# TORlN/HDR-to-SDR

Hardware: AMD Instinct MI355X
Metric: Mpixel/s HDR10->SDR (4K frames) at 1/2/4/8 GPUs; % HBM roofline (higher is better)
Workload: dtype f32

## Files before the change

hdr-to-sdr_amd/csrc/h2s_tile.h:

```cpp
#pragma once
#include "h2s_tile_io.h"

namespace h2s {

__device__ __forceinline__ CurveConsts curve_of(const CurveConsts* frames, int f) {
  typedef __attribute__((address_space(4))) const float cfloat;
  constexpr int n = (int)(sizeof(CurveConsts) / sizeof(float));
  cfloat* src = (cfloat*)frames + __builtin_amdgcn_readfirstlane(f) * n;
  CurveConsts r;
  float* dst = reinterpret_cast<float*>(&r);
#pragma unroll
  for (int i = 0; i < n; i++) dst[i] = src[i];
  return r;
}

constexpr int TILE_WPE = 5;
constexpr int TILE_WPE_LP = TILE_WPE;

template <int TRC, int TM, int DESAT, int LP, int DBG = 0, bool SEMI = false, int SUB = 0>
__global__ __launch_bounds__(256) __attribute__((amdgpu_waves_per_eu(LP ? TILE_WPE_LP : TILE_WPE))) void k_tile(
    const FastParams F) {
  static_assert(DBG == 0 || DBG == 1, "the stage is F.dbg_stage, not a template value");
  static_assert(SUB == 0 || SUB == 3 || (LP == 0 && DBG == 0), "4:2:2 / 4:4:4 input: CPU chain product instances only");
  static_assert(SUB != 3 || (DBG == 0 && SEMI), "top-left 4:2:0 input: the SEMI product instances");
  constexpr bool S420 = SUB == 0 || SUB == 3;
  constexpr int YST = row_stride<LP>(), HST = YST;
  static_assert(TBH * C422_ST <= (CBH + 2) * HST && TBH * C444_ST <= 2 * (CBH + 2) * HST, "hrow holds the SUB windows");
  __shared__ __attribute__((aligned(16))) unsigned char yin[YIN_BYTES];
  __shared__ float hrow[2][(CBH + 2) * HST];
  __shared__ float csum[2][CBH * CBW];
  __shared__ float4 pq_lds[PQ_NSEG + 1];
  __shared__ float4 pqi_lds[LP ? PQI_NTAB : 1];
  extern __shared__ uint16_t eq_lds[];
  __shared__ int tflag[2];
  __shared__ int offtab[4];
  __shared__ unsigned spread_lds[LP ? 256 : 1];
  constexpr int ESC = TRC == 0 || !LP ? PQ_SEG : 1;

  const int t = threadIdx.x;
  const int lane = t & 63, w = t >> 6;
  const unsigned ntiles = F.nbx * F.nby * F.nframes;
  unsigned tile = (unsigned)xcd_remap(blockIdx.x, gridDim.x) * (unsigned)F.tpb;
  const unsigned tend = tile + (unsigned)F.tpb < ntiles ? tile + (unsigned)F.tpb : ntiles;

  TileGeo geo = tile_geo(F, tile);
  const LaneOfs lofs = lane_ofs<SEMI>(F, t);
  TileRegs<SEMI, SUB> cur = tile_load<SEMI, SUB>(F, geo, t, lofs);
  const __amdgpu_buffer_rsrc_t req = __builtin_amdgcn_make_buffer_rsrc((void*)F.eq_lut, (short)0, 2 * F.eq_n, 0x00020000);
  const unsigned eq0 = __builtin_amdgcn_raw_buffer_load_b16(req, 2 * t, 0, 0);
  float4 pq0 = make_float4(0.0f, 0.0f, 0.0f, 0.0f);
  const bool stage_pq = TRC != 1 || !LP || F.lp_ipt;
  if (stage_pq && t < PQ_NSEG) {
    const __amdgpu_buffer_rsrc_t rpq = __builtin_amdgcn_make_buffer_rsrc((void*)F.pq_tab, (short)0, 16 * PQ_NSEG, 0x00020000);
    pq0 = __builtin_bit_cast(float4, __builtin_amdgcn_raw_buffer_load_b128(rpq, 16 * t, 0, 0));
  }
  const int eq_sh = SEMI ? F.out_sh : 0;
  if (t < F.eq_n) eq_lds[t] = (uint16_t)(((eq0 << F.shift_out) | (eq0 >> F.rep_rs)) << eq_sh);
  for (int i = t + 256; i < F.eq_n; i += 256) {
    const unsigned v = __builtin_amdgcn_raw_buffer_load_b16(req, 2 * i, 0, 0);
    eq_lds[i] = (uint16_t)(((v << F.shift_out) | (v >> F.rep_rs)) << eq_sh);
  }
  if (stage_pq && t < PQ_NSEG)
    pq_lds[t + 1] = (TRC == 0 || LP) && t == 0 ? make_float4(0.0f, 0.0f, 3.40282347e38f, 0.0f) : pq0;
  if (stage_pq && t == 255) pq_lds[0] = make_float4(0.0f, 0.0f, 0.0f, 0.0f);
  if (t < 2) tflag[t] = 0;
  if (t < 3) offtab[t] = t == 0 ? 12 : (t == 1 ? F.og : F.ob);
  if (LP) {
    unsigned x = (unsigned)t;
    x = (x | (x << 8)) & 0x0F00Fu;
    x = (x | (x << 4)) & 0x0C30C3u;
    spread_lds[t] = (x | (x << 2)) & 0x249249u;
  }
  __syncthreads();
  if (LP && (F.lp_ipt || TRC == 2)) {
    const __amdgpu_buffer_rsrc_t rpi = __builtin_amdgcn_make_buffer_rsrc((void*)F.pqi_tab, (short)0, 16 * PQI_NTAB, 0x00020000);
    for (int i = t; i < PQI_NTAB; i += 256)
      pqi_lds[i] = __builtin_bit_cast(float4, __builtin_amdgcn_raw_buffer_load_b128(rpi, 16 * i, 0, 0));
  }

  const int qx = (lane >> 2) & 3, qy = lane >> 4, pxl = lane & 1, pyl = (lane >> 1) & 1;
  const int xl = 16 * w + 2 * qx + pxl, yl = 2 * qy + pyl;
  uint16_t* ybase = reinterpret_cast<uint16_t*>(yin + luma_at(xl, yl));
  const float* h0 = hrow[0] + (qy + 1) * HST + xl;
  const float* h1 = hrow[1] + (qy + 1) * HST + xl;
  const int hb = SUB == 3 ? (pyl ? HST : 0) : (pyl ? HST : -HST);
  const float* c0 = hrow[0] + yl * C422_ST + (xl >> 1);
  const float* c1 = hrow[1] + yl * C422_ST + (xl >> 1);
  const int16_t* s0 = reinterpret_cast<const int16_t*>(hrow[0]) + yl * C444_ST + xl;
  const int16_t* s1 = reinterpret_cast<const int16_t*>(hrow[1]) + yl * C444_ST + xl;
  float* csb = csum[0] + qy * CBW + 8 * w + qx;

  const float yoff = in_vgpr(F.y_off_c) * (float)ESC + (ESC == PQ_SEG ? 1.0f : 0.0f);
  const float cmid = in_vgpr(F.c_mid);
  const float a_rv = in_vgpr(F.a_rv[1]) * (float)ESC, a_gv = in_vgpr(F.a_gv[1]) * (float)ESC,
              a_gu = in_vgpr(F.a_gu[1]) * (float)ESC, a_bu = in_vgpr(F.a_bu[1]) * (float)ESC;
  const float stride_g = in_vgpr(F.stride_g), stride_b = in_vgpr(F.stride_b);
  const int og = in_vgpr(F.og), ob = in_vgpr(F.ob), ocr = in_vgpr(F.cr), ocg = in_vgpr(F.cg), ocb = in_vgpr(F.cb);
  const float log2_nm1 = in_vgpr(F.log2_nm1), x_max = in_vgpr(F.x_max);
  const float ysc = in_vgpr(F.ys) * (float)ESC;
  const float ydq = F.dither ? dither_off(xl, yl) - 0.5f : 0.0f;
  const StepK K{a_rv, a_gv, a_gu, a_bu, stride_g, stride_b, og, ob, ocr, ocg, ocb, log2_nm1, x_max,
                TM == 5 && !LP ? in_vgpr(F.hable_kb) : F.hable_kb, F.c111, rintf(1.0f / F.inv_nm1), offtab,
                LP ? in_vgpr(F.lp_k2) : 0.0f, LP ? in_vgpr(F.lp_k2 + 255.0f) : 0.0f, LP ? F.lp_cy + ydq : 0.0f,
                LP ? in_vgpr(F.lp_k1) : 0.0f};
  gu32* lut8v = LP ? in_vgpr64(F.lut8x) : nullptr;
  float qo[4];
#pragma unroll
  for (int i = 0; i < 4; i++)
    qo[i] = LP ? F.lp_qo + (F.lp_dith ? bayer16(xl + 8 * (i & 1), yl + 8 * (i >> 1)) : 0.5f) -
                     (F.lut_off ? 0.0f : F.lp_k2 * F.lp_qs_f)
               : 0.5f;

  auto steps = [&](const TileGeo& g, auto fast) {
    constexpr bool FB = decltype(fast)::value;
    constexpr int YR2 = YROW / 2;
    if constexpr (FB) {
      H2S_MARK("body: fast");
    } else {
      H2S_MARK("body: exact-capable");
    }
    CurveConsts cv = F;
    if ((TM == 7 || TM == 8 || LP) && F.cv_frames) cv = curve_of(F.cv_frames, g.f);
    const CDoviRec* const dv =
        TRC == 2 ? (const CDoviRec*)F.dovi + __builtin_amdgcn_readfirstlane(F.dovi_n == 1 ? 0 : F.dovi_f0 + g.f) : nullptr;
    if constexpr (LP && TM == 7) {
      cv.b_e1b = in_vgpr(cv.b_e1b), cv.b_tb = in_vgpr(cv.b_tb), cv.b_c2 = in_vgpr(cv.b_c2);
      cv.b_lc = in_vgpr(cv.b_lc), cv.b_bk_b = in_vgpr(cv.b_bk_b), cv.b_bk_d = in_vgpr(cv.b_bk_d);
    } else if constexpr (LP && TM == 8) {
      cv.sp_qb_u = in_vgpr(cv.sp_qb_u), cv.sp_pb_u = in_vgpr(cv.sp_pb_u);
      cv.sp_srcmax = in_vgpr(cv.sp_srcmax), cv.sp_umax = in_vgpr(cv.sp_umax);
    }
    const __amdgpu_buffer_rsrc_t lut = __builtin_amdgcn_make_buffer_rsrc((void*)F.lut_yuv, (short)0, F.lut_bytes, 0x00020000);
    const int live = !FB && DBG == 0 && !F.chr444 ? F.H - g.py0 : TBH;
    auto chroma_out = [&](int s, float oyv, float ozv) {
      if (!FB && F.chr444) {
        const int px = g.px0 + xl + 8 * (s & 1), py = g.py0 + yl + 8 * (s >> 1);
        F.chr444[(long long)py * F.chr_w + px] = make_float2(oyv * F.inv_c56, ozv * F.inv_c56);
        return;
      }
      H2S_MARK("S6 chroma quad sums");
      const int oc = 4 * (s >> 1) * CBW + 4 * (s & 1);
      const float su = quad_sum(oyv), sv = quad_sum(ozv);
      csb[oc] = su;
      csb[oc + CBH * CBW] = sv;
    };
    if constexpr (LP && DBG == 0) {
      if (!F.lut_off) {
        unsigned vp = 0;
#pragma unroll
        for (int s = 0; s <= 8; s++) {
          unsigned vn = 0;
          if (s < 8 && (FB || 8 * (s >> 1) < live)) {
            const int oy = 8 * (s >> 1) * YR2 + 8 * (s & 1);
            const int oh = 4 * (s >> 1) * HST + 8 * (s & 1);
            H2S_MARK("S0 step: staged Y, vertical chroma");
            const float ybs = fmaf((float)ybase[oy], ysc, yoff);
            const float U = SUB == 3 ? 2.0f * (h0[oh] + h0[oh + hb]) : fmaf(3.0f, h0[oh], h0[oh + hb]);
            const float V = SUB == 3 ? 2.0f * (h1[oh] + h1[oh + hb]) : fmaf(3.0f, h1[oh], h1[oh + hb]);
            float r, gg, bl;
            lin_tone<TRC, TM, DESAT, LP, 0, FB>(F, cv, pq_lds, pqi_lds, K, ybs, U, V, [](float, float, float) {},
                                                 r, gg, bl, dv);
            H2S_MARK("S3 encode");
            vn = lp_table_read(F, K, lut8v, spread_lds, r, gg, bl, qo[s & 3]);
          }
          if (s > 0 && (FB || 8 * ((s - 1) >> 1) < live)) {
            const int sp = s - 1;
            const float R8 = (float)(vp & 255u), G8 = (float)((vp >> 8) & 255u), B8 = (float)((vp >> 16) & 255u);
            H2S_MARK("S5 Y'CbCr");
            const f3 o = lp_ycbcr(F, K, R8, G8, B8);
            H2S_MARK("S7 eq");
            ybase[8 * (sp >> 1) * YR2 + 8 * (sp & 1)] = eq_lds[(int)o.x];
            chroma_out(sp, o.y, o.z);
          }
          vp = vn;
        }
        return;
      }
      H2S_MARK("body: lut off");
    }
#pragma unroll
    for (int s = 0; s < 8; s++) {
      if (!FB && (s & 1) == 0 && 8 * (s >> 1) >= live) break;
      const int oy = 8 * (s >> 1) * YR2 + 8 * (s & 1);
      const int oh = 4 * (s >> 1) * HST + 8 * (s & 1);
      H2S_MARK("S0 step: staged Y, vertical chroma");
      const float ybs = fmaf((float)ybase[oy], ysc, yoff);
      float U, V;
      if constexpr (SUB == 1) {
        const int oc = 8 * (s >> 1) * C422_ST + 4 * (s & 1);
        U = 4.0f * (c0[oc] + c0[oc + pxl]), V = 4.0f * (c1[oc] + c1[oc + pxl]);
      } else if constexpr (SUB == 2) {
        const int oc = 8 * (s >> 1) * C444_ST + 8 * (s & 1);
        U = 8.0f * (float)s0[oc], V = 8.0f * (float)s1[oc];
      } else if constexpr (SUB == 3) {
        U = 2.0f * (h0[oh] + h0[oh + hb]), V = 2.0f * (h1[oh] + h1[oh + hb]);
      } else {
        U = fmaf(3.0f, h0[oh], h0[oh + hb]);
        V = fmaf(3.0f, h1[oh], h1[oh + hb]);
      }
      const long long di = DBG && g.f == 0 && g.py0 + yl + 8 * (s >> 1) < F.H
                               ? (long long)(g.py0 + yl + 8 * (s >> 1)) * F.dbg_w + g.px0 + xl + 8 * (s & 1)
                               : -1;
      float oyv, ozv;
      ybase[oy] = (uint16_t)px_chain<TRC, TM, DESAT, LP, DBG, FB>(
          F, cv, pq_lds, pqi_lds, eq_lds, lut8v, spread_lds, lut, K, ybs, U, V, di, oyv, ozv, LP ? qo[s & 3] : 0.5f, ydq, dv);
      chroma_out(s, oyv, ozv);
    }
  };
  auto mask_in = [&](uint4& a) {
    a.x &= F.in_mask2, a.y &= F.in_mask2, a.z &= F.in_mask2, a.w &= F.in_mask2;
  };
  auto shift_in = [&](uint4& a) { a.x >>= F.in_sh, a.y >>= F.in_sh, a.z >>= F.in_sh, a.w >>= F.in_sh; };

  const int pl = __builtin_amdgcn_readfirstlane(t >> 6) & 1, rem = t & 63;
  const bool cst = t < 128 && !F.chr444;
  auto commit = [&](unsigned ti) {
    H2S_MARK("tile: commit");
    if constexpr (SEMI && S420) {
      if (!F.in_semi) cur.uh = halo_half(F, geo, t, cur.uh);
    }
    if (F.in_mask2 != 0xFFFFFFFFu) {
      if constexpr (SEMI && S420) {
        if (F.in_sh) {
          shift_in(cur.ya), shift_in(cur.ua);
          cur.uh >>= F.in_sh;
        }
      }
      mask_in(cur.ya), mask_in(cur.ua);
      if constexpr (SUB == 2) mask_in(cur.va);
      else cur.uh &= F.in_mask2;
    }
    const float my = stage_luma(yin, cur.ya, t >> 3, t & 7, ysc, yoff);
    float mc = 0.0f;
    if constexpr (SUB == 1) {
      mc = stage_chroma422(hrow[__builtin_amdgcn_readfirstlane(t >> 7)], cur.ua, cur.uh, t & 127, cmid);
    } else if constexpr (SUB == 2) {
      mc = stage_chroma444(hrow[0], hrow[1], cur.ua, cur.va, t >> 3, t & 7, (int)F.c_mid);
    } else if (SEMI && F.in_semi) {
      if (t < 144) mc = stage_chroma_semi<HST>(hrow[0], hrow[1], cur.ua, cur.uh, t, cmid);
    } else if ((t & 127) < 72) {
      mc = stage_chroma<HST>(hrow[__builtin_amdgcn_readfirstlane(t >> 7)], cur.ua, cur.uh, t & 127, cmid);
    }
    if constexpr (SUB == 2) asm volatile("" ::"v"(cur.ua.w), "v"(cur.va.w));
    else asm volatile("" ::"v"(cur.ua.w), "v"(cur.uh));
    if ((my > F.safe_y || mc > F.safe_c)) tflag[ti & 1u] = 1;
  };
  commit(tile);
  for (;;) {
    H2S_MARK("tile: prefetch");
    const int par = (int)(tile & 1u);
    const TileGeo g = geo;
    const bool more = tile + 1 < tend;
    if (more) {
      tile_next(F, geo);
      cur = tile_load<SEMI, SUB>(F, geo, t, lofs);
    }
    __syncthreads();
    const bool fb = __builtin_amdgcn_readfirstlane(tflag[par]) == 0 && !F.chr444 && !(DBG == 0 && g.py0 + TBH > F.H);
    if (t == 0) tflag[par ^ 1] = 0;
    if (fb)
      steps(g, std::integral_constant<bool, true>{});
    else
      steps(g, std::integral_constant<bool, false>{});
    H2S_MARK("tile: store");
    __syncthreads();

    put_luma(F, g, read_luma(F, yin, t >> 3, t & 7), t >> 3, lofs.sy, t);
    const bool osemi = SEMI && F.out_semi;
    u4v cv{0u, 0u, 0u, 0u};
    int cvo = ST_DROP;
    if (cst) {
      const int cr = osemi ? t >> 3 : rem >> 2;
      cv = osemi ? read_chroma_semi(F, csum[0], cr, t & 7) : read_chroma(F, csum[0], pl, cr, rem & 3);
      if (g.cy0 + cr < F.ch) cvo = lofs.sc;
    }
    put_chroma(F, g, cv, osemi ? 0 : pl, osemi, cvo, t);
    if (!more) break;
    commit(++tile);
  }
}

}
```

hdr-to-sdr_amd/csrc/h2s_tile_io.h:

```cpp
#pragma once
#include "h2s_tile_px.h"

namespace h2s {

constexpr int CBW = 32, CBH = 16;
constexpr int ROW_STRIDE = 72, ROW_STRIDE_LP = 68;
template <int LP>
constexpr int row_stride() { return LP ? ROW_STRIDE_LP : ROW_STRIDE; }
constexpr int AUX_NT = 2;
constexpr int NT = AUX_NT, NTS = AUX_NT;

__device__ __forceinline__ void unpack8(const uint4 a, float* o) {
  o[0] = (float)(a.x & 0xffff), o[1] = (float)(a.x >> 16), o[2] = (float)(a.y & 0xffff), o[3] = (float)(a.y >> 16);
  o[4] = (float)(a.z & 0xffff), o[5] = (float)(a.z >> 16), o[6] = (float)(a.w & 0xffff), o[7] = (float)(a.w >> 16);
}

__device__ __forceinline__ __amdgpu_buffer_rsrc_t plane_rsrc(const uint8_t* base, int bytes) {
  return __builtin_amdgcn_make_buffer_rsrc((void*)base, (short)0, bytes, 0x00020000);
}

template <bool SEMI, int SUB = 0>
struct TileRegs {
  uint4 ya, ua;
  std::conditional_t<SEMI, unsigned, uint16_t> uh;
};
template <bool SEMI>
struct TileRegs<SEMI, 2> {
  uint4 ya, ua, va;
};

struct TileGeo {
  int f, px0, py0, cx0, cy0;
};

__device__ __forceinline__ TileGeo tile_geo(const FastParams& F, unsigned tile) {
  const unsigned bx = tile % F.nbx, bt = tile / F.nbx;
  TileGeo g;
  g.f = (int)(bt / F.nby);
  const int by = (int)(bt % F.nby);
  g.px0 = (int)bx * TBW, g.py0 = by * TBH, g.cx0 = (int)bx * CBW, g.cy0 = by * CBH;
  return g;
}

__device__ __forceinline__ void tile_next(const FastParams& F, TileGeo& g) {
  g.px0 += TBW, g.cx0 += CBW;
  if (g.px0 >= F.W) {
    g.px0 = 0, g.cx0 = 0, g.py0 += TBH, g.cy0 += CBH;
    if (g.py0 >= (int)F.nby * TBH) g.py0 = 0, g.cy0 = 0, g.f++;
  }
}

struct LaneOfs {
  int y, u;
  int sy, sc;
};

template <bool SEMI>
__device__ __forceinline__ LaneOfs lane_ofs(const FastParams& F, int t) {
  LaneOfs L;
  L.y = (t >> 3) * (int)F.in_ls[0] + 16 * (t & 7);
  const int pc = (t >> 7) & 1, tc = t & 127;
  L.u = (tc >> 2) * (int)F.in_ls[1 + pc] + 16 * (tc & 3);
  if (SEMI && F.in_semi) L.u = (t >> 3) * (int)F.in_ls[1] + 16 * (t & 7);
  const int sb = F.out8 ? 8 : 16;
  L.sy = (t >> 3) * (int)F.out_ls[0] + sb * (t & 7);
  const int pl = (t >> 6) & 1, rem = t & 63;
  L.sc = (rem >> 2) * (int)F.out_ls[1 + pl] + sb * (rem & 3);
  if (SEMI && F.out_semi) L.sc = (t >> 3) * (int)F.out_ls[1] + sb * (t & 7);
  return L;
}

template <bool SEMI, int SUB = 0>
__device__ __forceinline__ TileRegs<SEMI, SUB> tile_load(const FastParams& F, const TileGeo& g, int t, const LaneOfs& L) {
  const __amdgpu_buffer_rsrc_t iy = plane_rsrc(F.in[0] + g.f * F.in_fp[0], F.in_bytes[0]);
  const int yr = t >> 3, yc = t & 7;
  TileRegs<SEMI, SUB> r;
  int vy, sy;
  if (g.py0 + TBH <= F.H) {
    vy = L.y, sy = g.py0 * (int)F.in_ls[0] + 2 * g.px0;
  } else {
    vy = (g.py0 + yr < F.H ? g.py0 + yr : F.H - 1) * (int)F.in_ls[0] + 2 * (g.px0 + 8 * yc), sy = 0;
  }
  r.ya = __builtin_bit_cast(uint4, __builtin_amdgcn_raw_buffer_load_b128(iy, vy, sy, NT));
  if constexpr (SUB == 2) {
    const __amdgpu_buffer_rsrc_t iu = plane_rsrc(F.in[1] + g.f * F.in_fp[1], F.in_bytes[1]);
    const __amdgpu_buffer_rsrc_t iv = plane_rsrc(F.in[2] + g.f * F.in_fp[2], F.in_bytes[2]);
    const int lu = (int)F.in_ls[1], lv = (int)F.in_ls[2];
    int vu, vv, su, sv;
    if (g.py0 + TBH <= F.H) {
      vu = yr * lu + 16 * yc, vv = yr * lv + 16 * yc;
      su = g.py0 * lu + 2 * g.px0, sv = g.py0 * lv + 2 * g.px0;
    } else {
      const int row = g.py0 + yr < F.H ? g.py0 + yr : F.H - 1;
      vu = row * lu + 2 * (g.px0 + 8 * yc), vv = row * lv + 2 * (g.px0 + 8 * yc), su = sv = 0;
    }
    r.ua = __builtin_bit_cast(uint4, __builtin_amdgcn_raw_buffer_load_b128(iu, vu, su, NT));
    r.va = __builtin_bit_cast(uint4, __builtin_amdgcn_raw_buffer_load_b128(iv, vv, sv, NT));
    return r;
  } else if constexpr (SUB == 1) {
    const int pc = __builtin_amdgcn_readfirstlane(t >> 7), tc = t & 127;
    const __amdgpu_buffer_rsrc_t ic = plane_rsrc(F.in[1 + pc] + g.f * F.in_fp[1 + pc], F.in_bytes[1 + pc]);
    const int ls = (int)F.in_ls[1 + pc];
    int vc, vh, sc;
    if (g.py0 + TBH <= F.H && g.cx0 + CBW + 1 <= F.icw) {
      vc = L.u, vh = L.u + 16, sc = g.py0 * ls + 2 * g.cx0;
    } else {
      const int clr = tc >> 2, ccx = tc & 3;
      const int row = g.py0 + clr < F.H ? g.py0 + clr : F.H - 1;
      vc = row * ls + 2 * (g.cx0 + 8 * ccx);
      vh = row * ls + 2 * chroma_edge_at(g.cx0 + 8 * ccx + 8, F.icw, F.chroma_edge);
      sc = 0;
    }
    if ((tc & 3) != 3) vh = 0x7FFFFFF0;
    r.ua = __builtin_bit_cast(uint4, __builtin_amdgcn_raw_buffer_load_b128(ic, vc, sc, NT));
    r.uh = __builtin_amdgcn_raw_buffer_load_b16(ic, vh, sc, 0);
    return r;
  } else {
  const bool pair = SEMI && F.in_semi;
  int pc, vc, vh, sc;
  if (pair) {
    pc = 0;
    const int ls = (int)F.in_ls[1];
    if (g.cy0 >= 1 && g.cy0 + CBH + 1 <= F.ch && g.cx0 + CBW + 1 <= F.cw) {
      vc = L.u, vh = L.u + 16, sc = (g.cy0 - 1) * ls + 4 * g.cx0;
    } else {
      const int clr = t >> 3, ccx = t & 7;
      const int row = chroma_edge_at(g.cy0 - 1 + clr, F.ch, F.chroma_edge);
      vc = row * ls + 4 * (g.cx0 + 4 * ccx);
      vh = row * ls + 4 * chroma_edge_at(g.cx0 + 4 * ccx + 4, F.cw, F.chroma_edge);
      sc = 0;
    }
    if (t >= 144) vc = vh = 0x7FFFFFF0;
  } else {
    pc = __builtin_amdgcn_readfirstlane(t >> 7);
    const int tc = t & 127;
    const int ls = (int)F.in_ls[1 + pc];
    if (g.cy0 >= 1 && g.cy0 + CBH + 1 <= F.ch && g.cx0 + CBW + 1 <= F.cw) {
      vc = L.u, vh = L.u + 16, sc = (g.cy0 - 1) * ls + 2 * g.cx0;
    } else {
      const int clr = tc >> 2, ccx = tc & 3;
      const int row = chroma_edge_at(g.cy0 - 1 + clr, F.ch, F.chroma_edge);
      vc = row * ls + 2 * (g.cx0 + 8 * ccx);
      vh = row * ls + 2 * chroma_edge_at(g.cx0 + 8 * ccx + 8, F.cw, F.chroma_edge);
      sc = 0;
    }
    if (tc >= 72) vc = vh = 0x7FFFFFF0;
  }
  const __amdgpu_buffer_rsrc_t ic = plane_rsrc(F.in[1 + pc] + g.f * F.in_fp[1 + pc], F.in_bytes[1 + pc]);
  sc = __builtin_amdgcn_readfirstlane(sc);
  r.ua = __builtin_bit_cast(uint4, __builtin_amdgcn_raw_buffer_load_b128(ic, vc, sc, NT));
  if constexpr (SEMI) {
    r.uh = __builtin_amdgcn_raw_buffer_load_b32(ic, vh & ~2, sc, 0);
  } else {
    r.uh = __builtin_amdgcn_raw_buffer_load_b16(ic, vh, sc, 0);
  }
  return r;
  }
}

__device__ __forceinline__ unsigned halo_half(const FastParams& F, const TileGeo& g, int t, unsigned hw) {
  int hs = 0;
  if (!(g.cy0 >= 1 && g.cy0 + CBH + 1 <= F.ch && g.cx0 + CBW + 1 <= F.cw))
    hs = (chroma_edge_at(g.cx0 + 8 * (t & 3) + 8, F.cw, F.chroma_edge) & 1) << 4;
  return (hw >> hs) & 0xffffu;
}

constexpr int YROW = 144;
constexpr int luma_at(int x, int y) { return y * YROW + 2 * x; }
static_assert(YROW % 16 == 0 && luma_at(8, 0) == 16, "a chunk of 8 samples is one aligned 16-byte slot");
static_assert(luma_at(0, 1) >= luma_at(TBW - 1, 0) + 2, "the rows' slots are disjoint");
static_assert((luma_at(0, 1) / 4) % 32 == 4 && luma_at(7, 0) / 4 == 3, "a step's 8 rows x 4 dwords cover the 32 banks once");
constexpr int YIN_BYTES = luma_at(0, TBH);
typedef unsigned short us2v __attribute__((ext_vector_type(2)));
__device__ __forceinline__ float stage_luma(unsigned char* yin, uint4 a, int row, int col8, float ysc, float yoff) {
  *reinterpret_cast<uint4*>(yin + luma_at(8 * col8, row)) = a;
  const us2v m = __builtin_elementwise_max(
      __builtin_elementwise_max(__builtin_bit_cast(us2v, a.x), __builtin_bit_cast(us2v, a.y)),
      __builtin_elementwise_max(__builtin_bit_cast(us2v, a.z), __builtin_bit_cast(us2v, a.w)));
  return fmaf((float)(m.x > m.y ? m.x : m.y), ysc, yoff);
}
template <int HST>
__device__ __forceinline__ float stage_chroma(float* plane, uint4 a, unsigned h, int tt, float cmid) {
  float v[9];
  unpack8(a, v);
  v[8] = (float)h;
#pragma unroll
  for (int k = 0; k < 9; k++) v[k] -= cmid;
  float m = fabsf(v[0]);
#pragma unroll
  for (int k = 1; k < 9; k++) m = __builtin_fmaxf(m, fabsf(v[k]));
  float* d = plane + (tt >> 2) * HST + 16 * (tt & 3);
#pragma unroll
  for (int k = 0; k < 4; k++)
    *reinterpret_cast<float4*>(d + 4 * k) =
        make_float4(v[2 * k] + v[2 * k], v[2 * k] + v[2 * k + 1], v[2 * k + 1] + v[2 * k + 1], v[2 * k + 1] + v[2 * k + 2]);
  return m;
}
template <int HST>
__device__ __forceinline__ float stage_chroma_semi(float* plane_u, float* plane_v, uint4 a, unsigned h, int tt, float cmid) {
  const unsigned w[5] = {a.x, a.y, a.z, a.w, h};
  float u[5], v[5];
#pragma unroll
  for (int k = 0; k < 5; k++) u[k] = (float)(w[k] & 0xffff) - cmid, v[k] = (float)(w[k] >> 16) - cmid;
  float m = __builtin_fmaxf(fabsf(u[0]), fabsf(v[0]));
#pragma unroll
  for (int k = 1; k < 5; k++) m = __builtin_fmaxf(m, __builtin_fmaxf(fabsf(u[k]), fabsf(v[k])));
  const int o = (tt >> 3) * HST + 8 * (tt & 7);
#pragma unroll
  for (int k = 0; k < 2; k++) {
    *reinterpret_cast<float4*>(plane_u + o + 4 * k) =
        make_float4(u[2 * k] + u[2 * k], u[2 * k] + u[2 * k + 1], u[2 * k + 1] + u[2 * k + 1], u[2 * k + 1] + u[2 * k + 2]);
    *reinterpret_cast<float4*>(plane_v + o + 4 * k) =
        make_float4(v[2 * k] + v[2 * k], v[2 * k] + v[2 * k + 1], v[2 * k + 1] + v[2 * k + 1], v[2 * k + 1] + v[2 * k + 2]);
  }
  return m;
}
constexpr int C422_ST = 36;
constexpr int C444_ST = 72;
__device__ __forceinline__ float stage_chroma422(float* plane, uint4 a, unsigned h, int tt, float cmid) {
  float v[9];
  unpack8(a, v);
  v[8] = (float)h;
#pragma unroll
  for (int k = 0; k < 9; k++) v[k] -= cmid;
  float m = fabsf(v[0]);
#pragma unroll
  for (int k = 1; k < 8; k++) m = __builtin_fmaxf(m, fabsf(v[k]));
  float* d = plane + (tt >> 2) * C422_ST + 8 * (tt & 3);
  *reinterpret_cast<float4*>(d) = make_float4(v[0], v[1], v[2], v[3]);
  *reinterpret_cast<float4*>(d + 4) = make_float4(v[4], v[5], v[6], v[7]);
  if ((tt & 3) == 3) d[8] = v[8], m = __builtin_fmaxf(m, fabsf(v[8]));
  return m;
}
__device__ __forceinline__ float stage_chroma444(float* plane_u, float* plane_v, uint4 a, uint4 b, int row, int col8,
                                                 int imid) {
  auto pack = [&](uint4 q, float* plane, float& m) {
    const unsigned w[4] = {q.x, q.y, q.z, q.w};
    unsigned o[4];
#pragma unroll
    for (int k = 0; k < 4; k++) {
      const int lo = (int)(w[k] & 0xffff) - imid, hi = (int)(w[k] >> 16) - imid;
      m = __builtin_fmaxf(m, __builtin_fmaxf(fabsf((float)lo), fabsf((float)hi)));
      o[k] = ((unsigned)lo & 0xffffu) | ((unsigned)hi << 16);
    }
    *reinterpret_cast<uint4*>(reinterpret_cast<int16_t*>(plane) + row * C444_ST + 8 * col8) = make_uint4(o[0], o[1], o[2], o[3]);
  };
  float m = 0.0f;
  pack(a, plane_u, m);
  pack(b, plane_v, m);
  return m;
}
__device__ __forceinline__ u4v read_luma(const FastParams& F, const unsigned char* yin, int r, int c) {
  const uint4 a = *reinterpret_cast<const uint4*>(yin + luma_at(8 * c, r));
  if (F.out8)
    return u4v{__builtin_amdgcn_perm(a.y, a.x, 0x06040200u), __builtin_amdgcn_perm(a.w, a.z, 0x06040200u), 0u, 0u};
  return u4v{a.x, a.y, a.z, a.w};
}
constexpr int ST_DROP = (int)0x80000000u;
__device__ __forceinline__ void tile_store(const FastParams& F, u4v v, __amdgpu_buffer_rsrc_t rs, int vo, int so, int t) {
  if (F.out8) {
    v.z = (unsigned)__builtin_amdgcn_update_dpp(0, (int)v.x, 0xB1, 0xF, 0xF, false);
    v.w = (unsigned)__builtin_amdgcn_update_dpp(0, (int)v.y, 0xB1, 0xF, 0xF, false);
    if (t & 1) vo = ST_DROP;
  }
  __builtin_amdgcn_raw_buffer_store_b128(v, rs, vo, so, NTS);
}
__device__ __forceinline__ void put_luma(const FastParams& F, const TileGeo& g, u4v v, int r, int vo, int t) {
  if (g.py0 + r >= F.H) vo = ST_DROP;
  const __amdgpu_buffer_rsrc_t oy_ = plane_rsrc(F.out[0] + g.f * F.out_fp[0], F.out_bytes[0]);
  tile_store(F, v, oy_, vo, g.py0 * (int)F.out_ls[0] + (F.out8 ? g.px0 : 2 * g.px0), t);
}
__device__ __forceinline__ u4v read_chroma(const FastParams& F, const float* csum, int pl, int r, int c) {
  const float4* src = reinterpret_cast<const float4*>(csum + pl * (CBH * CBW) + r * CBW + 8 * c);
  const float4 v0 = src[0], v1 = src[1];
  const float vv[8] = {v0.x, v0.y, v0.z, v0.w, v1.x, v1.y, v1.z, v1.w};
  unsigned code[8];
  if (F.dither) {
#pragma unroll
    for (int k = 0; k < 8; k++) code[k] = (unsigned)(int)(vv[k] + (F.c_bias - 0.5f + dither_off(k, r)));
  } else {
#pragma unroll
    for (int k = 0; k < 8; k++) code[k] = (unsigned)(int)(vv[k] + F.c_bias);
  }
  if (F.rep_rs == 31) {
#pragma unroll
    for (int k = 0; k < 8; k++) code[k] <<= F.shift_out;
  } else {
#pragma unroll
    for (int k = 0; k < 8; k++) code[k] = (code[k] << F.shift_out) | (code[k] >> F.rep_rs);
  }
  if (F.out8)
    return u4v{code[0] | (code[1] << 8) | (code[2] << 16) | (code[3] << 24),
               code[4] | (code[5] << 8) | (code[6] << 16) | (code[7] << 24), 0u, 0u};
  return u4v{code[0] | (code[1] << 16), code[2] | (code[3] << 16), code[4] | (code[5] << 16), code[6] | (code[7] << 16)};
}
__device__ __forceinline__ void put_chroma(const FastParams& F, const TileGeo& g, u4v v, int pl, bool semi, int vo, int t) {
  const __amdgpu_buffer_rsrc_t oc_ = plane_rsrc(F.out[1 + pl] + g.f * F.out_fp[1 + pl], F.out_bytes[1 + pl]);
  tile_store(F, v, oc_, vo, g.cy0 * (int)F.out_ls[1 + pl] + ((F.out8 ? g.cx0 : 2 * g.cx0) << (semi ? 1 : 0)), t);
}

__device__ __forceinline__ u4v read_chroma_semi(const FastParams& F, const float* csum, int r, int c) {
  const float4 vu = *reinterpret_cast<const float4*>(csum + r * CBW + 4 * c);
  const float4 vv = *reinterpret_cast<const float4*>(csum + CBH * CBW + r * CBW + 4 * c);
  const float s[8] = {vu.x, vv.x, vu.y, vv.y, vu.z, vv.z, vu.w, vv.w};
  unsigned code[8];
  if (F.dither) {
#pragma unroll
    for (int k = 0; k < 8; k++) code[k] = (unsigned)(int)(s[k] + (F.c_bias - 0.5f + dither_off(4 * (c & 1) + (k >> 1), r)));
  } else {
#pragma unroll
    for (int k = 0; k < 8; k++) code[k] = (unsigned)(int)(s[k] + F.c_bias);
  }
  if (F.rep_rs == 31) {
#pragma unroll
    for (int k = 0; k < 8; k++) code[k] <<= F.shift_out;
  } else {
#pragma unroll
    for (int k = 0; k < 8; k++) code[k] = (code[k] << F.shift_out) | (code[k] >> F.rep_rs);
  }
  if (F.out8)
    return u4v{code[0] | (code[1] << 8) | (code[2] << 16) | (code[3] << 24),
               code[4] | (code[5] << 8) | (code[6] << 16) | (code[7] << 24), 0u, 0u};
  return u4v{(code[0] | (code[1] << 16)) << F.out_sh, (code[2] | (code[3] << 16)) << F.out_sh,
             (code[4] | (code[5] << 16)) << F.out_sh, (code[6] | (code[7] << 16)) << F.out_sh};
}

}
```

Before: 275,700.

## Remap non-LP wave footprint to 2D blocks and tile chroma-sum LDS layout

```diff
diff --git a/hdr-to-sdr_amd/csrc/h2s_tile.h b/hdr-to-sdr_amd/csrc/h2s_tile.h
--- a/hdr-to-sdr_amd/csrc/h2s_tile.h
+++ b/hdr-to-sdr_amd/csrc/h2s_tile.h
@@ -78,17 +78,21 @@
       pqi_lds[i] = __builtin_bit_cast(float4, __builtin_amdgcn_raw_buffer_load_b128(rpi, 16 * i, 0, 0));
   }
 
+  constexpr bool MB = !LP;
+  auto SX = [](int s) { return MB ? 16 * (s & 3) : 8 * (s & 1); };
+  auto SY = [](int s) { return MB ? 16 * (s >> 2) : 8 * (s >> 1); };
+  const int wx = MB ? w & 1 : 2 * w, wy = MB ? __builtin_amdgcn_readfirstlane(w >> 1) : 0;
   const int qx = (lane >> 2) & 3, qy = lane >> 4, pxl = lane & 1, pyl = (lane >> 1) & 1;
-  const int xl = 16 * w + 2 * qx + pxl, yl = 2 * qy + pyl;
+  const int xl = 8 * wx + 2 * qx + pxl, yl = 8 * wy + 2 * qy + pyl;
   uint16_t* ybase = reinterpret_cast<uint16_t*>(yin + luma_at(xl, yl));
-  const float* h0 = hrow[0] + (qy + 1) * HST + xl;
-  const float* h1 = hrow[1] + (qy + 1) * HST + xl;
+  const float* h0 = hrow[0] + ((yl >> 1) + 1) * HST + xl;
+  const float* h1 = hrow[1] + ((yl >> 1) + 1) * HST + xl;
   const int hb = SUB == 3 ? (pyl ? HST : 0) : (pyl ? HST : -HST);
   const float* c0 = hrow[0] + yl * C422_ST + (xl >> 1);
   const float* c1 = hrow[1] + yl * C422_ST + (xl >> 1);
   const int16_t* s0 = reinterpret_cast<const int16_t*>(hrow[0]) + yl * C444_ST + xl;
   const int16_t* s1 = reinterpret_cast<const int16_t*>(hrow[1]) + yl * C444_ST + xl;
-  float* csb = csum[0] + qy * CBW + 8 * w + qx;
+  float* csb = csum[0] + csum_at(xl >> 1, yl >> 1);
 
   const float yoff = in_vgpr(F.y_off_c) * (float)ESC + (ESC == PQ_SEG ? 1.0f : 0.0f);
   const float cmid = in_vgpr(F.c_mid);
@@ -107,7 +111,7 @@
   float qo[4];
 #pragma unroll
   for (int i = 0; i < 4; i++)
-    qo[i] = LP ? F.lp_qo + (F.lp_dith ? bayer16(xl + 8 * (i & 1), yl + 8 * (i >> 1)) : 0.5f) -
+    qo[i] = LP ? F.lp_qo + (F.lp_dith ? bayer16(xl + SX(i), yl + SY(i)) : 0.5f) -
                      (F.lut_off ? 0.0f : F.lp_k2 * F.lp_qs_f)
                : 0.5f;
 
@@ -131,15 +135,15 @@
       cv.sp_srcmax = in_vgpr(cv.sp_srcmax), cv.sp_umax = in_vgpr(cv.sp_umax);
     }
     const __amdgpu_buffer_rsrc_t lut = __builtin_amdgcn_make_buffer_rsrc((void*)F.lut_yuv, (short)0, F.lut_bytes, 0x00020000);
-    const int live = !FB && DBG == 0 && !F.chr444 ? F.H - g.py0 : TBH;
+    const int live = !FB && DBG == 0 && !F.chr444 ? F.H - g.py0 - 8 * wy : TBH;
     auto chroma_out = [&](int s, float oyv, float ozv) {
       if (!FB && F.chr444) {
-        const int px = g.px0 + xl + 8 * (s & 1), py = g.py0 + yl + 8 * (s >> 1);
+        const int px = g.px0 + xl + SX(s), py = g.py0 + yl + SY(s);
         F.chr444[(long long)py * F.chr_w + px] = make_float2(oyv * F.inv_c56, ozv * F.inv_c56);
         return;
       }
       H2S_MARK("S6 chroma quad sums");
-      const int oc = 4 * (s >> 1) * CBW + 4 * (s & 1);
+      const int oc = csum_at(SX(s) / 2, SY(s) / 2);
       const float su = quad_sum(oyv), sv = quad_sum(ozv);
       csb[oc] = su;
       csb[oc + CBH * CBW] = sv;
@@ -150,9 +154,9 @@
 #pragma unroll
         for (int s = 0; s <= 8; s++) {
           unsigned vn = 0;
-          if (s < 8 && (FB || 8 * (s >> 1) < live)) {
-            const int oy = 8 * (s >> 1) * YR2 + 8 * (s & 1);
-            const int oh = 4 * (s >> 1) * HST + 8 * (s & 1);
+          if (s < 8 && (FB || SY(s) < live)) {
+            const int oy = SY(s) * YR2 + SX(s);
+            const int oh = SY(s) / 2 * HST + SX(s);
             H2S_MARK("S0 step: staged Y, vertical chroma");
             const float ybs = fmaf((float)ybase[oy], ysc, yoff);
             const float U = SUB == 3 ? 2.0f * (h0[oh] + h0[oh + hb]) : fmaf(3.0f, h0[oh], h0[oh + hb]);
@@ -163,13 +167,13 @@
             H2S_MARK("S3 encode");
             vn = lp_table_read(F, K, lut8v, spread_lds, r, gg, bl, qo[s & 3]);
           }
-          if (s > 0 && (FB || 8 * ((s - 1) >> 1) < live)) {
+          if (s > 0 && (FB || SY(s - 1) < live)) {
             const int sp = s - 1;
             const float R8 = (float)(vp & 255u), G8 = (float)((vp >> 8) & 255u), B8 = (float)((vp >> 16) & 255u);
             H2S_MARK("S5 Y'CbCr");
             const f3 o = lp_ycbcr(F, K, R8, G8, B8);
             H2S_MARK("S7 eq");
-            ybase[8 * (sp >> 1) * YR2 + 8 * (sp & 1)] = eq_lds[(int)o.x];
+            ybase[SY(sp) * YR2 + SX(sp)] = eq_lds[(int)o.x];
             chroma_out(sp, o.y, o.z);
           }
           vp = vn;
@@ -180,17 +184,17 @@
     }
 #pragma unroll
     for (int s = 0; s < 8; s++) {
-      if (!FB && (s & 1) == 0 && 8 * (s >> 1) >= live) break;
-      const int oy = 8 * (s >> 1) * YR2 + 8 * (s & 1);
-      const int oh = 4 * (s >> 1) * HST + 8 * (s & 1);
+      if (!FB && SX(s) == 0 && SY(s) >= live) break;
+      const int oy = SY(s) * YR2 + SX(s);
+      const int oh = SY(s) / 2 * HST + SX(s);
       H2S_MARK("S0 step: staged Y, vertical chroma");
       const float ybs = fmaf((float)ybase[oy], ysc, yoff);
       float U, V;
       if constexpr (SUB == 1) {
-        const int oc = 8 * (s >> 1) * C422_ST + 4 * (s & 1);
+        const int oc = SY(s) * C422_ST + SX(s) / 2;
         U = 4.0f * (c0[oc] + c0[oc + pxl]), V = 4.0f * (c1[oc] + c1[oc + pxl]);
       } else if constexpr (SUB == 2) {
-        const int oc = 8 * (s >> 1) * C444_ST + 8 * (s & 1);
+        const int oc = SY(s) * C444_ST + SX(s);
         U = 8.0f * (float)s0[oc], V = 8.0f * (float)s1[oc];
       } else if constexpr (SUB == 3) {
         U = 2.0f * (h0[oh] + h0[oh + hb]), V = 2.0f * (h1[oh] + h1[oh + hb]);
@@ -198,8 +202,8 @@
         U = fmaf(3.0f, h0[oh], h0[oh + hb]);
         V = fmaf(3.0f, h1[oh], h1[oh + hb]);
       }
-      const long long di = DBG && g.f == 0 && g.py0 + yl + 8 * (s >> 1) < F.H
-                               ? (long long)(g.py0 + yl + 8 * (s >> 1)) * F.dbg_w + g.px0 + xl + 8 * (s & 1)
+      const long long di = DBG && g.f == 0 && g.py0 + yl + SY(s) < F.H
+                               ? (long long)(g.py0 + yl + SY(s)) * F.dbg_w + g.px0 + xl + SX(s)
                                : -1;
       float oyv, ozv;
       ybase[oy] = (uint16_t)px_chain<TRC, TM, DESAT, LP, DBG, FB>(
diff --git a/hdr-to-sdr_amd/csrc/h2s_tile_io.h b/hdr-to-sdr_amd/csrc/h2s_tile_io.h
--- a/hdr-to-sdr_amd/csrc/h2s_tile_io.h
+++ b/hdr-to-sdr_amd/csrc/h2s_tile_io.h
@@ -4,6 +4,10 @@
 namespace h2s {
 
 constexpr int CBW = 32, CBH = 16;
+constexpr int csum_at(int cx, int cy) { return (cx >> 3) * (CBH * 8) + cy * 8 + (cx & 7); }
+static_assert(csum_at(8, 0) * 4 % 256 == 0 && csum_at(0, 8) * 4 % 256 == 0 && CBH * CBW * 4 % 256 == 0,
+              "a step's and the plane's offsets are whole 256-byte units");
+static_assert(csum_at(CBW - 1, CBH - 1) == CBH * CBW - 1, "csum_at fills the plane");
 constexpr int ROW_STRIDE = 72, ROW_STRIDE_LP = 68;
 template <int LP>
 constexpr int row_stride() { return LP ? ROW_STRIDE_LP : ROW_STRIDE; }
@@ -271,7 +275,7 @@
   tile_store(F, v, oy_, vo, g.py0 * (int)F.out_ls[0] + (F.out8 ? g.px0 : 2 * g.px0), t);
 }
 __device__ __forceinline__ u4v read_chroma(const FastParams& F, const float* csum, int pl, int r, int c) {
-  const float4* src = reinterpret_cast<const float4*>(csum + pl * (CBH * CBW) + r * CBW + 8 * c);
+  const float4* src = reinterpret_cast<const float4*>(csum + pl * (CBH * CBW) + csum_at(8 * c, r));
   const float4 v0 = src[0], v1 = src[1];
   const float vv[8] = {v0.x, v0.y, v0.z, v0.w, v1.x, v1.y, v1.z, v1.w};
   unsigned code[8];
@@ -300,8 +304,8 @@
 }
 
 __device__ __forceinline__ u4v read_chroma_semi(const FastParams& F, const float* csum, int r, int c) {
-  const float4 vu = *reinterpret_cast<const float4*>(csum + r * CBW + 4 * c);
-  const float4 vv = *reinterpret_cast<const float4*>(csum + CBH * CBW + r * CBW + 4 * c);
+  const float4 vu = *reinterpret_cast<const float4*>(csum + csum_at(4 * c, r));
+  const float4 vv = *reinterpret_cast<const float4*>(csum + CBH * CBW + csum_at(4 * c, r));
   const float s[8] = {vu.x, vv.x, vu.y, vv.y, vu.z, vv.z, vu.w, vv.w};
   unsigned code[8];
   if (F.dither) {
```

After: 279,100, median of 6. 1.01x the previous value.
